# TimD1/vcfdist

Measured on AMD Instinct MI355X. Metric: supercluster-alignments/sec, higher is better.
Workload: dtype int32; 1 GPU; wgs_synth; superclusters_per_gpu=1000000, span_dist=lognormal(median 20, sigma 1.2) clip [4,10000]

## Files before the change

### vcfdist_amd/csrc/pr_api.hip

```cpp
#include <hip/hip_runtime.h>
#include <hip/hip_ext.h>
#include <dlfcn.h>

#include <algorithm>
#include <atomic>
#include <chrono>
#include <cstdarg>
#include <cstdio>
#include <cstdlib>
#include <cstring>
#include <condition_variable>
#include <deque>
#include <functional>
#include <mutex>
#include <string>
#include <thread>
#include <tuple>
#include <unordered_map>
#include <unordered_set>
#include <vector>

#include "../../include/vcfdist_pr.h"
#include "pr_device.h"
#include "pr_plan.h"
// ... 199 lines not shown
    if (lane == 0) wcnt[wave] = npop;
    __syncthreads();
    if (threadIdx.x == 0) {
        const int tot = wcnt[0] + wcnt[1] + wcnt[2] + wcnt[3];
        const int totp = pad4 ? ((tot + 3) & ~3) : tot;
        wbase = totp ? atomicAdd(cnt, totp) : 0;
        wtot = tot; wpad = totp - tot;
    }
    __syncthreads();
    int base = wbase;
    for (int w = 0; w < wave; w++) base += wcnt[w];
    if (bad) fail_list[base + __popcll(mbad & ((1ull << lane) - 1ull))] = a;
    if (int(threadIdx.x) < wpad) fail_list[wbase + wtot + int(threadIdx.x)] = -1;
}

__global__ void k_fails_count(const int32_t *__restrict__ work, int n, const AlnOut *__restrict__ outs, int32_t *__restrict__ blk,
                              int pad4, const int32_t *__restrict__ n_dev) {
    if (n_dev) n = min(n, *n_dev);
    const int i = blockIdx.x * blockDim.x + threadIdx.x;
    const int a = i < n ? work[i] : -1;
    const bool bad = a >= 0 && !outs[a].band_ok;
    const int npop = __popcll(__ballot(bad));
    __shared__ int wcnt[4];
    if ((threadIdx.x & 63) == 0) wcnt[threadIdx.x >> 6] = npop;
    __syncthreads();
    if (threadIdx.x == 0) {
        const int tot = wcnt[0] + wcnt[1] + wcnt[2] + wcnt[3];
        blk[blockIdx.x] = pad4 ? ((tot + 3) & ~3) : tot;
    }
}

#define FAILS_SCAN_NT 256
__global__ void __launch_bounds__(FAILS_SCAN_NT) k_fails_scan(int32_t *__restrict__ blk, int nb, int32_t *__restrict__ cnt) {
    __shared__ int32_t s_sum[FAILS_SCAN_NT];
    const int tid = threadIdx.x;
    const int per = (nb + FAILS_SCAN_NT - 1) / FAILS_SCAN_NT;
    const int b = min(nb, tid * per), e = min(nb, b + per);
    int32_t sum = 0;
    for (int k = b; k < e; k++) sum += blk[k];
    s_sum[tid] = sum;
    __syncthreads();
    for (int o = 1; o < FAILS_SCAN_NT; o <<= 1) {
        const int32_t v = tid >= o ? s_sum[tid - o] : 0;
        __syncthreads();
        s_sum[tid] += v;
        __syncthreads();
    }
    int32_t off = s_sum[tid] - sum;
    for (int k = b; k < e; k++) { const int32_t c = blk[k]; blk[k] = off; off += c; }
    if (tid == FAILS_SCAN_NT - 1) *cnt = s_sum[FAILS_SCAN_NT - 1];
}

__global__ void k_fails_scatter(const int32_t *__restrict__ work, int n, const AlnOut *__restrict__ outs, const int32_t *__restrict__ blk,
                                int32_t *__restrict__ fail_list, int pad4, const int32_t *__restrict__ n_dev) {
    if (n_dev) n = min(n, *n_dev);
    const int i = blockIdx.x * blockDim.x + threadIdx.x;
    const int a = i < n ? work[i] : -1;
    const bool bad = a >= 0 && !outs[a].band_ok;
    const unsigned long long mbad = __ballot(bad);
    const int lane = threadIdx.x & 63, wave = threadIdx.x >> 6;
    __shared__ int wcnt[4];
    if (lane == 0) wcnt[wave] = __popcll(mbad);
    __syncthreads();
    const int tot = wcnt[0] + wcnt[1] + wcnt[2] + wcnt[3];
    const int totp = pad4 ? ((tot + 3) & ~3) : tot;
    const int wbase = blk[blockIdx.x];
    int base = wbase;
    for (int w = 0; w < wave; w++) base += wcnt[w];
    if (bad) fail_list[base + __popcll(mbad & ((1ull << lane) - 1ull))] = a;
    if (int(threadIdx.x) < totp - tot) fail_list[wbase + tot + int(threadIdx.x)] = -1;
}

__global__ void k_publish_fails(const int32_t *__restrict__ list, const int32_t *__restrict__ cnt, int32_t *__restrict__ h_list,
                                int32_t *__restrict__ h_cnt, int copy_list) {
    const int n = *cnt;
    if (copy_list)
        for (int i = blockIdx.x * blockDim.x + threadIdx.x; i < n; i += gridDim.x * blockDim.x) h_list[i] = list[i];
    if (blockIdx.x == 0 && threadIdx.x == 0) *h_cnt = n;
    __threadfence_system();
}
// ... 6 lines not shown
    const AlnDesc d = src[i];
    dst[d.sc * 4 + d.aln] = d;
    dst_work[i] = src_work[i];
}

__global__ void k_collect_ties(const AlnOut *__restrict__ outs, int n, int4 *__restrict__ list, int32_t *__restrict__ cnt, int cap) {
    const int i = blockIdx.x * blockDim.x + threadIdx.x;
    if (i >= n) return;
    const int b = outs[i].band_ok;
    if (b >= 0) return;
    const int k = atomicAdd(cnt, 1);
    if (k < cap) list[k] = make_int4(i, -b - 1, outs[i].n_sec, outs[i].s);
}

__global__ void k_collect_ties_list(const int32_t *__restrict__ work, int n, const AlnOut *__restrict__ outs, int4 *__restrict__ list,
                                    int32_t *__restrict__ cnt, int cap) {
    const int i = blockIdx.x * blockDim.x + threadIdx.x;
    if (i >= n) return;
    const int a = work[i];
    if (a < 0) return;
    const int b = outs[a].band_ok;
    if (b >= 0) return;
    const int k = atomicAdd(cnt, 1);
    if (k < cap) list[k] = make_int4(a, -b - 1, outs[a].n_sec, outs[a].s);
}
__global__ void k_collect_spec(const int32_t *__restrict__ work, int n, const AlnOut *__restrict__ outs, int tag, int4 *__restrict__ list,
                               int32_t *__restrict__ cnt, int cap) {
    const int i = blockIdx.x * blockDim.x + threadIdx.x;
    if (i >= n) return;
    const int a = work[i];
    if (a < 0) return;
// ... 1344 lines not shown
    double phase_ms[6] = {0, 0, 0, 0, 0, 0};
    void phase(int k) { phase_ms[k] = std::chrono::duration<double, std::milli>(std::chrono::steady_clock::now() - call0).count(); }
    void lapx(const char *what) {
        if (h->debug) fprintf(stderr, "[vpr] execute %-34s %8.3f ms\n", what,
                              std::chrono::duration<double, std::milli>(std::chrono::steady_clock::now() - wall0).count());
    }

    void post_flag(int idx, hipStream_t ks) {
        flag_exp[idx] = ++h->flag_seq;
        hipLaunchKernelGGL(k_flag, dim3(1), dim3(1), 0, ks, h->hp_flag + idx, flag_exp[idx]);
        const hipError_t e = hipGetLastError();
        if (e != hipSuccess && launch_err == hipSuccess) launch_err = e;
    }
    hipError_t launch_err = hipSuccess;
    int64_t zl_wave0 = 0, zl_rows = 0;

    int idle_check(int64_t idle_polls, std::chrono::steady_clock::time_point since) {
        if (launch_err != hipSuccess) return fail(h, VPR_ERR_DEVICE, "kernel launch failed: %s", hipGetErrorString(launch_err));
        if (idle_polls % 2048) return VPR_OK;
        hipStream_t ss[] = {h->stream, h->cls_stream[0], h->cls_stream[1], h->cls_stream[2], h->cls_stream[3], h->cls_stream[4],
                            h->cls_stream[5], h->cls_stream[6], h->cls_stream[7],
                            h->tie_stream[0], h->tie_stream[1], h->tie_stream[2], h->tie_stream[3]};
        bool busy = false;
        for (hipStream_t s_ : ss) {
            const hipError_t e = hipStreamQuery(s_);
            if (e != hipSuccess && e != hipErrorNotReady) return fail(h, VPR_ERR_DEVICE, "stream error while waiting for a round: %s", hipGetErrorString(e));
            busy = busy || e == hipErrorNotReady;
        }
        const double idle_s = std::chrono::duration<double>(std::chrono::steady_clock::now() - since).count();
        static const double limit_s = [] { const char *e = getenv("VPR_IDLE_TIMEOUT_S"); const double v = e ? atof(e) : 0.0; return v > 0 ? v : 1800.0; }();
// ... 441 lines not shown
            restore = true;
            for (int32_t k = 0; k < cnt && restore; k++) {
                const auto it = tie_early.find(P.work[size_t(off) + size_t(k)]);
                if (it == tie_early.end() || it->second.plan != &h->plan0 || (it->second.mode != 1 && it->second.mode != 3) ||
                    it->second.pos < tie_resident->work_off || it->second.pos >= tie_resident->work_off + tie_resident->n_long) { restore = false; break; }
                const AlnDesc od = plan_desc(h, h->plan0, size_t(it->second.pos)), nd = plan_desc(h, P, size_t(off) + size_t(k));
                if (od.band_pad != LV_TAG[LV_C1] || od.pitch[0] != nd.pitch[0] || od.pitch[1] != nd.pitch[1] ||
                    od.mat_off[1] + int64_t(od.pitch[1]) * od.Lt > h->save_bytes) { restore = false; break; }
                rjobs[k] = RestoreJob{{od.mat_off[0], od.mat_off[1]}, od.blo_off};
            }
        }
        rc = timed(1, ls, ks, restore ? "k_restore_stripe" : band_fwd_name(lv), [&] {
            if (zero)
                hipExtLaunchKernelGGL(k_zero_lane, dim3((cnt + 63) / 64), dim3(64), h->zl_lds_bytes, ks, own_a, own_b, 0, h->d_descs, list, cnt,
                                      h->d_zl_hdr + zl_wave0, h->d_zl_in, h->d_zl_log, h->d_outs, a_path,
                                      (h->cfg.flags & VPR_CFG_KEEP_PATHS) ? 1 : 0, h->d_d1_hdr ? h->d1_max_rows : 0, h->lane_prio_rows);
            else if (q16)
                hipLaunchKernelGGL(k_fwd_q16, dim3((cnt + 3) / 4), dim3(64), 0, ks, h->dB, h->d_descs, list, cnt,
                                   P.arena, a_i32, h->d_outs, n_dev);
            else if (restore)
                hipLaunchKernelGGL(k_restore_stripe, dim3(cnt), dim3(256), 0, ks, h->d_descs, list, rjobs, h->plan0.arena,
                                   int64_t(reinterpret_cast<intptr_t>(h->d_save) - reinterpret_cast<intptr_t>(h->plan0.arena)), P.arena, a_i32);
            else if (save)
                hipLaunchKernelGGL(k_fwd_stripe_save, dim3(cnt), dim3(64), 0, ks, h->dB, h->d_descs, list, P.arena, a_i32, h->d_outs,
                                   fwd_save_delta);
            else
                hipLaunchKernelGGL(band_fwd_kernel(lv), dim3(cnt), dim3(lv >= LV_C4 ? W : 64), 0,
                                   ks, h->dB, h->d_descs, list, P.arena, a_i32, h->d_outs);
            hipLaunchKernelGGL(k_fwd_band_finish, dim3((cnt + 255) / 256), dim3(256), 0, ks, list, cnt, h->d_outs, tag, n_dev);
        }, zero);
        if (rc) return rc;
        n_fwd++;
        {
            const int32_t nc = n_dev ? n_all : cnt;
            if (zero && h->d_d1_blk) ordered_fails(list, nc, h->d_fail + fail_off, h->d_cnt + slot, n_dev, ks);
            else
            hipLaunchKernelGGL(k_collect_fails, dim3((nc + 255) / 256), dim3(256), 0, ks, list, nc, h->d_outs,
                               h->d_fail + fail_off, h->d_cnt + slot, zero ? 1 : 0, n_dev);
            hipLaunchKernelGGL(k_publish_fails, dim3(zero ? 1 : std::min((nc + 255) / 256, 1024)), dim3(256), 0, ks,
                               h->d_fail + fail_off, h->d_cnt + slot, h->hp_fail + fail_off, h->hp_cnt + slot, zero ? 0 : 1);
        }
        HIPCHK(h, hipEventRecord(h->ev_slot[slot], ks));
        }
        if ((phases & 2) && !zero) {
        ls.bytes_algorithmic = ls.cells;
        rc = timed(2, ls, ks, band_bwd_name(lv), [&] {
            if (q16)
                hipLaunchKernelGGL(k_bwd_q16, dim3((cnt + 3) / 4), dim3(64), 0, ks, h->dB, h->d_descs, list, cnt,
                                   P.arena, a_i32, h->d_outs, tag, dtag, n_dev);
            else
                hipLaunchKernelGGL(band_bwd_kernel(lv), dim3(cnt), dim3(lv >= LV_C4 ? W : 64), 0,
                                   ks, h->dB, h->d_descs, list, P.arena, a_i32, h->d_outs, tag);
        });
        if (rc) return rc;
        }
// ... 97 lines not shown
                if (wave_credit)
                    hipLaunchKernelGGL(k_credit<true>, dim3(cnt), dim3(64), 0, ks, h->dB, h->d_descs, list, cnt,
                                       h->d_outs, a_path, h->d_secs, h->d_fp_table, h->d_jobs, h->d_njobs,
                                       h->jobs_cap, dtag, tag, n_dev);
                else
                    hipLaunchKernelGGL(k_credit<false>, dim3((cnt + 63) / 64), dim3(64), 0, ks, h->dB, h->d_descs,
                                       list, cnt, h->d_outs, a_path, h->d_secs, h->d_fp_table, h->d_jobs,
                                       h->d_njobs, h->jobs_cap, dtag, tag, n_dev);
            });
        } else {
            rc = walk_launch(P, list, cnt, ks, wave_walk, tag);
        }
        return rc;
    }

    void ordered_fails(const int32_t *list, int32_t nc, int32_t *out, int32_t *cnt, const int32_t *n_dev, hipStream_t ks) {
        const int nb = (nc + 255) / 256;
        hipLaunchKernelGGL(k_fails_count, dim3(nb), dim3(256), 0, ks, list, nc, h->d_outs, h->d_d1_blk, 1, n_dev);
        hipLaunchKernelGGL(k_fails_scan, dim3(1), dim3(FAILS_SCAN_NT), 0, ks, h->d_d1_blk, nb, cnt);
        hipLaunchKernelGGL(k_fails_scatter, dim3(nb), dim3(256), 0, ks, list, nc, h->d_outs, h->d_d1_blk, out, 1, n_dev);
    }

    int enqueue_d1(const int32_t *list, const int32_t *n_dev, int32_t cap, int32_t n_all, hipStream_t ks, int ph, int ztag) {
        const int nw = (cap + 63) / 64;
        vpr_launch_stat ls;
        memset(&ls, 0, sizeof(ls));
        ls.threads = 64; ls.cells_per_thread = 1; ls.n_units = cap;
        int rc = VPR_OK;
        if (ph == 1) {
            rc = timed(0, ls, ks, "k_prep_d1", [&] {
                hipLaunchKernelGGL(k_d1_hdr, dim3(nw), dim3(64), 0, ks, h->d_descs, list, n_dev, cap, h->d_outs, h->d_d1_hdr);
                hipLaunchKernelGGL(k_d1_scan, dim3(1), dim3(D1_SCAN_NT), 0, ks, h->d_d1_hdr, nw, h->d1_in_cap, h->d1_log_cap, h->d_d1_info);
                hipLaunchKernelGGL(k_prep_d1, dim3(nw), dim3(256), 0, ks, h->dB, h->d_descs, list, n_dev, cap, h->d_outs, h->d_d1_hdr, h->d_d1_in);
            });
            if (rc) return rc;
            rc = timed(1, ls, ks, "k_one_lane", [&] {
                hipLaunchKernelGGL(k_one_lane, dim3(nw), dim3(64), 0, ks, h->d_descs, list, n_dev, cap, h->d_d1_hdr, h->d_d1_in, h->d_d1_log,
                                   h->d_outs, reinterpret_cast<PathEnt *>(h->plan0.arena), (h->cfg.flags & VPR_CFG_KEEP_PATHS) ? 1 : 0, h->d_d1_info,
                                   std::max(1, h->lane_prio_rows / 4));
                hipLaunchKernelGGL(k_fwd_band_finish, dim3((cap + 255) / 256), dim3(256), 0, ks, list, cap, h->d_outs, D1_TAG, n_dev);
            });
            if (rc) return rc;
            ordered_fails(list, n_all, h->d_d1_fail, h->d_d1_info + 2, n_dev, ks);
        } else if (ph == 4) {
            ls.cells_per_thread = 3;
            rc = timed(3, ls, ks, "k_one_tail", [&] {
                hipLaunchKernelGGL(k_one_tail, dim3(nw), dim3(64), 0, ks, h->dB, h->d_descs, list, n_dev, cap, h->d_d1_hdr, h->d_d1_in, h->d_d1_log,
                                   h->d_outs, reinterpret_cast<PathEnt *>(h->plan0.arena), (h->cfg.flags & VPR_CFG_KEEP_PATHS) ? 1 : 0, h->d_d1_info,
                                   h->d_secs, h->d_fp_table, h->d_jobs, h->d_njobs, h->jobs_cap, ztag, std::max(1, h->lane_prio_rows / 4));
            });
        }
        return rc;
    }

    int read_fails(int slot, int64_t fail_off, hipStream_t ls, std::vector<int32_t> &fails) {
        HIPCHK(h, x_event_sync(h, h->ev_slot[slot], SITE));
        const int32_t nf = h->hp_cnt[slot];
        if (nf > 0) {
// ... 26 lines not shown
            if (rc) return rc;
        }
        c.pending.clear();
        c.plans.clear();
        c.slot_cur = 0; c.fail_cur = 0;
        if (!overlap(c)) { c.stage_cur = 0; c.arena_cur = 0; }
        return VPR_OK;
    }

    int lad_tie_off(int k) { return h->tie_list_cap / 2 + k * (h->tie_list_cap / 4); }

    int lad_tie_cap(int k) { (void)k; return h->tie_list_cap / 4; }

    void ladder_collect(int k, const int32_t *list, int32_t n, hipStream_t ks) {
        hipLaunchKernelGGL(k_collect_ties_list, blocks(n), dim3(256), 0, ks, list, n, h->d_outs, h->d_tie_list + lad_tie_off(k),
                           h->d_tie_cnt + 5 + k, lad_tie_cap(k));
        hipLaunchKernelGGL(k_publish_ties, dim3(4), dim3(256), 0, ks, h->d_tie_list + lad_tie_off(k), h->d_tie_cnt + 5 + k,
                           h->hp_tie_list + lad_tie_off(k), h->hp_tie_cnt + 5 + k, lad_tie_cap(k));
        post_flag(9 + k, ks);
        lad_tie_wait[k] = true;
    }

    void drop_resident(const LadderCtx &c) {
        for (auto &r : h->resident)
            if (r.second >= c.arena && r.second < c.arena + c.arena_bytes) r.second = nullptr;
    }

    bool lad_grow(LadderCtx &c, int64_t nb, int64_t must = 0) {
        const int k = int(&c - h->lad);
        for (int j = 0; j < 4; j++) {
            LadderCtx &g = h->lad[j];
// ... 267 lines not shown
        tie_full = false;
        if (h->debug) fprintf(stderr, "[vpr] speculative replays: %d long alignments\n", n);
        int rc_ = tie_replay(spec_plan, 0, n, LT.ls, true);
        if (rc_) return rc_;
        spec_slot = tie_patch_slot; spec_off = tie_patch_off; spec_cap = tie_patch_cap;
        tie_patch_slot = -1;
        HIPCHK(h, hipEventRecord(h->ev_spec, LT.ls2));
        (void)hipStreamQuery(LT.ls2);
        for (int32_t k = 0; k < n; k++) spec_set[lst[k].x] = 1;
        tie_early.clear();
        tie_job_blocks.emplace_back(h->hp_tie_jobs + j0, tie_job_cur - j0);
        tie_job_total += tie_job_cur - j0;
        return VPR_OK;
    }

    int collect_part(int k, const int32_t *list, int32_t n, hipStream_t ks) {
        hipLaunchKernelGGL(k_collect_ties_list, blocks(n), dim3(256), 0, ks, list, n, h->d_outs, h->d_tie_list + tie_off[k],
                           h->d_tie_cnt + 2 + k, tie_cap[k]);
        hipLaunchKernelGGL(k_publish_ties, dim3(4), dim3(256), 0, ks, h->d_tie_list + tie_off[k], h->d_tie_cnt + 2 + k,
                           h->hp_tie_list + tie_off[k], h->hp_tie_cnt + 2 + k, tie_cap[k]);
        post_flag(2 + k, ks);
        return VPR_OK;
    }

    int round0_windowed() {
        int rc = VPR_OK;
        LL.ls = h->cls_stream[2]; LS.ls = h->cls_stream[3];
        LL.ls2 = h->cls_stream[5]; LS.ls2 = h->cls_stream[6]; LL.ev2 = h->ev_side[0]; LS.ev2 = h->ev_side[1];
        LL.slot0 = 2; LS.slot0 = 2 + LadderCtx::N_SLOTS;
        for (size_t ci = 0; ci < P0.chunks.size(); ci++) {
            const Chunk &ch = P0.chunks[ci];
            const int32_t n_long = ch.n_long;
            LL.arena_cur = LS.arena_cur = 0; LL.stage_cur = LS.stage_cur = 0;
            const int64_t rbase = na_ + na_ / 16 + 256;
            LL.fail_base = rbase; LS.fail_base = rbase + n_long;
            HIPCHK(h, hipMemsetAsync(h->d_cnt, 0, 8, st));
            if (ci == 0 && h->d_d1_info) HIPCHK(h, hipMemsetAsync(h->d_d1_info, 0, 64, st));
            HIPCHK(h, hipMemsetAsync(h->d_tie_cnt, 0, 32, st));
            HIPCHK(h, hipMemsetAsync(h->d_tie_ndec, 0, TIE_DEC_SLOTS * 4, st));
            tie_dec_slot = 0; tie_dec_cur = 0; tie_patch_slot = -1; spec_slot = -1;
            HIPCHK(h, hipEventRecord(h->ev_fork, st));
            HIPCHK(h, hipStreamWaitEvent(s_long, h->ev_fork, 0));
            HIPCHK(h, hipStreamWaitEvent(s_short, h->ev_fork, 0));
            HIPCHK(h, hipStreamWaitEvent(LL.ls, h->ev_fork, 0));
            HIPCHK(h, hipStreamWaitEvent(LS.ls, h->ev_fork, 0));
            for (int k = 0; k < 4; k++) HIPCHK(h, hipStreamWaitEvent(h->tie_stream[k], h->ev_fork, 0));
            for (int k = 2; k < 4; k++)
                for (int e = 0; e < 2; e++) {
                    LadderCtx &c = h->lad[k];
                    c.tie_clean[e] = 0;
                    if (ci == 0 && c.tie_scratch[e] && c.tie_first[e] > 0 && c.tie_first[e] <= c.tie_scratch_bytes[e]) {
// ... 11 lines not shown
            const bool inplace = P0.lv == LV_Z && n_short > 0;
            const int32_t *short_list = P0.d_work + ch.work_off + n_long;
            if (n_short > 0 && !inplace) {
                for (int ph = 1; ph <= 4; ph <<= 1) {
                    if ((rc = enqueue_part(P0, P0.d_work, ch.work_off + n_long, n_short, P0.lv, s_short, 1, n_long, false,
                                           ch.part_cells[1], ch.part_in[1], ch.part_dense[1], -1, ph))) return rc;
                    if (ph == 1) post_flag(1, s_short);
                    if (ph == 2 && (rc = collect_part(1, short_list, n_short, s_short))) return rc;
                }
            }
            if (inplace) {
                zl_wave0 = h->zl_wave0[ci];
                zl_rows = ch.part_rows[1];
                const int32_t *n_dev = h->d_cnt + 1;
                const int ztag = LV_TAG[LV_Z];
                HIPCHK(h, hipMemsetAsync(h->d_cnt + SLOT_IP, 0, 4, s_short));
                const bool d1 = h->d_d1_hdr != nullptr && cap_ip <= h->d1_wave_cap * 64;
                const int32_t n_all1 = n_short + n_short / 16 + 64;
                if (d1) HIPCHK(h, hipMemsetAsync(h->d_d1_info + 2, 0, 4, s_short));
                hipStream_t s_cred = h->side_credit ? h->cls_stream[7] : s_short;
                for (int ph = 1; ph <= 4; ph <<= 1) {
                    if (ph != 4 || s_cred == s_short) {
                        if ((rc = enqueue_part(P0, P0.d_work, ch.work_off + n_long, n_short, LV_Z, s_short, 1, n_long, false,
                                               ch.part_cells[1], ch.part_in[1], ch.part_dense[1], -1, ph))) return rc;
                        if (d1 && (rc = enqueue_d1(h->d_fail + n_long, n_dev, cap_ip, n_all1, s_short, ph, ztag))) return rc;
                    }
                    if (ph == 1 && s_cred != s_short) {
                        HIPCHK(h, hipEventRecord(h->ev_cred[0], s_short));
                        HIPCHK(h, hipStreamWaitEvent(s_cred, h->ev_cred[0], 0));
                        if ((rc = enqueue_part(P0, P0.d_work, ch.work_off + n_long, n_short, LV_Z, s_cred, 1, n_long, false,
                                               ch.part_cells[1], ch.part_in[1], ch.part_dense[1], -1, 4))) return rc;
                        if (d1 && (rc = enqueue_d1(h->d_fail + n_long, n_dev, cap_ip, n_all1, s_cred, 4, ztag))) return rc;
                        HIPCHK(h, hipEventRecord(h->ev_cred[1], s_cred));
                    }
                    if (ph == 4 && s_cred != s_short) HIPCHK(h, hipStreamWaitEvent(s_short, h->ev_cred[1], 0));
                    if ((rc = d1 ? enqueue_part(P0, h->d_d1_fail, 0, cap_ip, LV_Q16, s_short, SLOT_IP, foff_ip, false, 0, 0, 0,
                                                ztag, ph, h->d_d1_info + 2, std::min<int32_t>(h->d1_fail_cap, n_all1 + n_all1 / 64 + 64))
                                 : enqueue_part(P0, h->d_fail, n_long, cap_ip, LV_Q16, s_short, SLOT_IP, foff_ip, false, 0, 0, 0,
                                                ztag, ph, n_dev, n_all1))) return rc;
                    if (ph == 1) post_flag(1, s_short);
                    if (ph == 2 && (rc = collect_part(1, short_list, n_short, s_short))) return rc;
                }
            }
            if (n_long > 0) {
                const int lv = P0.lv <= LV_Q16 ? LONG_LV : P0.lv;
                for (int ph = 1; ph <= 4; ph <<= 1) {
                    fwd_save_delta = (ph == 1 && lv == LV_C1 && h->d_save) ? int64_t(reinterpret_cast<intptr_t>(h->d_save) - reinterpret_cast<intptr_t>(P0.arena)) : 0;
                    rc = enqueue_part(P0, P0.d_work, ch.work_off, n_long, lv, s_long, 0, 0, true, ch.part_cells[0],
                                      ch.part_in[0], ch.part_dense[0], -1, ph);
                    fwd_save_delta = 0;
                    if (rc) return rc;
                    if (ph == 1) {
                        post_flag(0, s_long);
                        if (lv == LV_C1) {
                            hipLaunchKernelGGL(k_collect_spec, blocks(n_long), dim3(256), 0, s_long, P0.d_work + ch.work_off, n_long, h->d_outs,
                                               LV_TAG[LV_C1], h->d_tie_list + tie_off[2], h->d_tie_cnt + 4, tie_cap[2]);
// ... 481 lines not shown
```

### vcfdist_amd/csrc/pr_d1.hip

```cpp
#ifndef PR_D1_HIP_
#define PR_D1_HIP_

#define D1_TAG 9
#define D1_CLEAN ZL_CLEAN_REJECT

#define GE_ALIVE 1u
#define GE_MAT 2u
#define GE_SWP 4u
#define GE_PSLOT_SHIFT 3
#define GE_SUB 32u
#define GE_SUB_SHIFT 6
#define GE_INS 256u
#define GE_INS_SHIFT 9
#define GE_DEL 2048u
#define GE_DEL_SHIFT 12
#define GE_TP 16384u
#define GE_BWD 32768u

#define MV_SWP_R 0
#define MV_MAT 1
#define MV_SUB 2
#define MV_INS 3
#define MV_DEL 4
#define MV_SWP_Q 5
// ... 124 lines not shown
                tile[lane][l] = v;
            }
            __syncthreads();
            const int rows = min(64, mlen - x0);
            for (int r = sub; r < rows; r += 4) out[int64_t(x0 + r) * 64 + lane] = tile[r][lane];
            __syncthreads();
        }
        out += int64_t(mlen) * 64;
    }
}

__global__ void __launch_bounds__(64, 3) k_one_lane(const AlnDesc *__restrict__ descs, const int32_t *__restrict__ list,
                                                    const int32_t *__restrict__ n_dev, int n_cap, const ZlWave *__restrict__ hdr,
                                                    const uint32_t *__restrict__ zin, uint4 *__restrict__ zlog,
                                                    AlnOut *__restrict__ outs, PathEnt *__restrict__ paths, int keep_paths,
                                                    int32_t *__restrict__ info, int prio_rows) {
    const int w = blockIdx.x, lane = threadIdx.x;
    const ZlWave H = hdr[w];
    if (H.mt <= 0) return;
    if (H.mt >= prio_rows) __builtin_amdgcn_s_setprio(2);
    const int n_list = min(*n_dev, n_cap);
    const int wi = w * 64 + lane;
    int a_ = wi < n_list ? list[wi] : -1;
    if (a_ >= 0 && outs[a_].exit_min != D1_CLEAN) a_ = -1;
    const bool live = a_ >= 0;
    {
        const int nl = __popcll(__ballot(live));
        if (lane == 0 && nl) atomicAdd(info + 3, nl);
    }
    const int a = max(a_, 0);
    const AlnDesc *dp = descs + a;
    const int Lq = live ? dp->Lq : 1, Lr = live ? dp->Lr : 1, Lt = live ? dp->Lt : 0;
    const int L[2] = {Lq, Lr};
    const auto rin = __builtin_amdgcn_make_buffer_rsrc(const_cast<uint32_t *>(zin + H.in_off), 0, 256 * (2 * H.mq + 2 * H.mr + H.mt), 0x00020000);
    const auto rlog = __builtin_amdgcn_make_buffer_rsrc(zlog + H.log_off, 0, 2560 * (H.mt + 1), 0x00020000);
    const uint32_t lane4 = uint32_t(lane) << 2, lane8 = uint32_t(lane) << 3, lane16 = uint32_t(lane) << 4;
    const uint32_t posW[2] = {0u, uint32_t(2 * H.mq) << 8}, posC[2] = {uint32_t(H.mq) << 8, uint32_t(2 * H.mq + H.mr) << 8};
    const uint32_t post = uint32_t(2 * H.mq + 2 * H.mr) << 8;
    const uint32_t logB1 = uint32_t(H.mt + 1) << 10, logB2 = logB1 + (uint32_t(H.mt + 1) << 9);
    auto in_at = [&](uint32_t off) -> uint32_t { return __builtin_amdgcn_raw_buffer_load_b32(rin, off, 0, 0); };
    auto word_at = [&](int p, int x, bool on) -> uint32_t { return in_at(on ? posW[p] + (uint32_t(x) << 8) + lane4 : ZL_OOB); };
    auto t_at = [&](int t, bool on) -> uint32_t { return in_at(on ? post + (uint32_t(t) << 8) + lane4 : ZL_OOB); };
    bool ok = live && Lt >= 2;
    const int rows = ok ? Lt : 0;
    int tmax = rows;
#pragma unroll
    for (int o = 32; o; o >>= 1) tmax = max(tmax, __shfl_xor(tmax, o));
    if (tmax == 0) return;
    using S2 = std::integral_constant<int, 2>;
    using S4 = std::integral_constant<int, 4>;
#ifdef D1_CLOCKS
    long long ck0 = wall_clock64();
    auto lapck = [&](int k) { const long long c = wall_clock64(); if (lane == 0) { atomicMax(info + 8 + k, int(c - ck0)); } ck0 = c; };
#else
    auto lapck = [&](int) {};
#endif

    int brow0 = 1 << 30;
    {
        int bq[2][4];
#pragma unroll
        for (int p = 0; p < 2; p++) {
#pragma unroll
// ... 78 lines not shown
            if (!__any(act)) continue;
            const uint32_t tw1 = t_at(t, act), tw0 = t_at(t - 1, act);
            const bool upper = act && (bq[0][2] >= 0 || bq[0][3] >= 0 || bq[1][2] >= 0 || bq[1][3] >= 0);
#ifdef D1_CLOCKS
            n_rows_++;
            if (__any(upper)) n_s4_++;
#endif
            if (__any(upper) || !b0_row(S2{}, t, act, tw1, tw0)) (void)b0_row(S4{}, t, act, tw1, tw0);
        }
#ifdef D1_CLOCKS
        if (lane == 0) { atomicAdd(info + 12, n_rows_); atomicAdd(info + 13, n_s4_); }
#endif
    }
    { const int c_ = __popcll(__ballot(ok)); if (lane == 0 && c_) atomicAdd(info + 5, c_); }
    lapck(0);
    if (!__any(ok)) return;

    {
        int fq[2][4], gq[2][4];
        uint32_t fw[2][4], gw[2][4];
#pragma unroll
        for (int p = 0; p < 2; p++) {
#pragma unroll
            for (int s = 0; s < 4; s++) { fq[p][s] = -1; fw[p][s] = 0; gq[p][s] = -1; gw[p][s] = 0; }
        }
        uint32_t tw0 = 0;
        auto fg_row = [&](auto Sc, int t, bool act, uint32_t tw1, const zl_u4 bp) -> bool {
            constexpr int S = decltype(Sc)::value;
            const uint32_t Tb = ZW_BASE(tw1);
            const bool t_allow = zw_fwd_allow(tw0);
            int nq[2][S];
// ... 152 lines not shown
            const zl_u4 bp = bp_n;
            bp_n = b_row(t + 1);
            tw_n = t_at(t + 1, ok && t + 1 < rows);
            bool upper = act && ((bp.y | bp.w) != 0u);
#pragma unroll
            for (int p = 0; p < 2; p++) upper = upper || (act && (fq[p][2] >= 0 || fq[p][3] >= 0 || gq[p][2] >= 0 || gq[p][3] >= 0));
            if (__any(upper) || !fg_row(S2{}, t, act, tw1, bp)) (void)fg_row(S4{}, t, act, tw1, bp);
        }
        { const int c_ = __popcll(__ballot(ok)); if (lane == 0 && c_) atomicAdd(info + 6, c_); }
        ok = ok && gq[0][0] == Lq - 1;
        { const int c_ = __popcll(__ballot(ok)); if (lane == 0 && c_) atomicAdd(info + 7, c_); }
    }
    lapck(1);
    if (live) {
        AlnOut &o = outs[a];
        o.dist_q = ok ? 1 : D_INF;
        o.dist_r = D_INF;
        o.exit_min = ok ? D_INF : 0;
    }
    if (!__any(ok)) return;

    const int nrow = ok ? Lt : 0;
    int bmax = nrow;
#pragma unroll
    for (int o = 32; o; o >>= 1) bmax = max(bmax, __shfl_xor(bmax, o));
    int beg_plane = VPR_PLANE_REF;
    {
        int kf[2][4], kg[2][4];
        uint32_t cf[2] = {0, 0};
        uint32_t cg[2][2] = {{0, 0}, {0, 0}};
#pragma unroll
        for (int p = 0; p < 2; p++) {
#pragma unroll
// ... 253 lines not shown
```

### vcfdist_amd/csrc/pr_zl.hip

```cpp
#ifndef PR_ZL_HIP_
#define PR_ZL_HIP_
#include <type_traits>


#define ZW_PTR(w) (int((w) & 0xffffu) - 1)
#define ZW_BASE(w) (((w) >> 16) & 0x7fu)
#define ZW_PV (1u << 23)
#define ZW_PB (1u << 24)
#define ZW_PE (1u << 25)
#define ZW_INS (1u << 26)
#define ZW_TP (1u << 27)
__device__ __forceinline__ bool zw_fwd_allow(uint32_t w) { return !(w & ZW_PV) || (w & ZW_PE); }
__device__ __forceinline__ bool zw_bwd_allow(uint32_t w) { return !(w & ZW_PV) || (w & ZW_PB); }

#define ZE_ALIVE 1u
#define ZE_HASMAT 2u
#define ZE_HASSWP 4u
#define ZE_PSLOT_SHIFT 3
#define ZE_TP 32u
#define ZE_BWD 64u

#define ZL_MAXLEN 65000
#define ZL_CLEAN_REJECT (-1)

// ... 53 lines not shown
            const int rows = min(64, mlen - x0);
            for (int r = sub; r < rows; r += 4) out[int64_t(x0 + r) * 64 + lane] = tile[r][lane];
            __syncthreads();
        }
        out += int64_t(mlen) * 64;
    }
}

typedef __attribute__((ext_vector_type(4))) unsigned int zl_u4;
typedef __attribute__((ext_vector_type(2))) unsigned int zl_u2;
#define ZL_OOB 0xfffffff0u

__global__ void __launch_bounds__(64, 6) k_zero_lane(const AlnDesc *__restrict__ descs, const int32_t *__restrict__ list, int n_list,
                                                  const ZlWave *__restrict__ hdr, const uint32_t *__restrict__ zin,
                                                  uint4 *__restrict__ zlog, AlnOut *__restrict__ outs, PathEnt *__restrict__ paths,
                                                  int keep_paths, int d1_max_rows, int prio_rows) {
    const int w = blockIdx.x, lane = threadIdx.x;
    const ZlWave H = hdr[w];
    if (H.mt >= prio_rows) __builtin_amdgcn_s_setprio(2);
    const int wi = w * 64 + lane;
    const int a_ = wi < n_list ? list[wi] : -1;
    const bool live = a_ >= 0;
    const int a = max(a_, 0);
    const AlnDesc *dp = descs + a;
    const int Lq = live ? dp->Lq : 1, Lr = live ? dp->Lr : 1, Lt = live ? dp->Lt : 0;
    const int L[2] = {Lq, Lr};
    const auto rin = __builtin_amdgcn_make_buffer_rsrc(const_cast<uint32_t *>(zin + H.in_off), 0, 256 * (H.mq + H.mr + H.mt), 0x00020000);
    const auto rlog = __builtin_amdgcn_make_buffer_rsrc(zlog + H.log_off, 0, 1280 * H.mt, 0x00020000);
    const uint32_t lane4 = uint32_t(lane) << 2, lane8 = uint32_t(lane) << 3;
    const uint32_t pos0[2] = {0u, uint32_t(H.mq) << 8}, post = uint32_t(H.mq + H.mr) << 8;
    const uint32_t logP0 = uint32_t(H.mt) << 9;
    auto in_at = [&](uint32_t off) -> uint32_t { return __builtin_amdgcn_raw_buffer_load_b32(rin, off, 0, 0); };
    bool ok = live && Lq < ZL_MAXLEN && Lr < ZL_MAXLEN && Lt < ZL_MAXLEN && Lt >= 2;
    const int rows = ok ? Lt : 0;
    int tmax = rows;
#pragma unroll
    for (int o = 32; o; o >>= 1) tmax = max(tmax, __shfl_xor(tmax, o));
    if (tmax == 0) {
        if (live) { outs[a].dist_q = D_INF; outs[a].dist_r = D_INF; outs[a].exit_min = 0; }
        return;
    }

    int qri[2][4];
    uint32_t pw[2][4];
#pragma unroll
    for (int p = 0; p < 2; p++) {
#pragma unroll
        for (int s = 0; s < 4; s++) { qri[p][s] = -1; pw[p][s] = 0; }
    }
    uint32_t tw0 = in_at(ok ? post + lane4 : ZL_OOB);
    if (ok) {
        qri[0][0] = 0; pw[0][0] = in_at(pos0[0] + lane4);
        qri[1][0] = 0; pw[1][0] = in_at(pos0[1] + lane4);
        zl_u2 e0;
// ... 107 lines not shown
#pragma unroll
        for (int p = 0; p < 2; p++) upper = upper || (act && (qri[p][2] >= 0 || qri[p][3] >= 0));
        if (__any(upper) || !fwd_row(std::integral_constant<int, 2>{}, t, act, tw1))
            (void)fwd_row(std::integral_constant<int, 4>{}, t, act, tw1);
    }
    int endq = -1, endr = -1;
#pragma unroll
    for (int s = 0; s < 4; s++) {
        if (qri[0][s] == Lq - 1) endq = s;
        if (qri[1][s] == Lr - 1) endr = s;
    }
    const bool clean = ok && Lt <= d1_max_rows;
    ok = ok && (endq >= 0 || endr >= 0);
    if (live) {
        AlnOut &o = outs[a];
        o.dist_q = (ok && endq >= 0) ? 0 : D_INF;
        o.dist_r = (ok && endr >= 0) ? 0 : D_INF;
        o.exit_min = ok ? D_INF : (clean ? ZL_CLEAN_REJECT : 0);
    }
    if (!__any(ok)) return;

    const int nrow = ok ? Lt : 0;
    int sc[2][4];
#pragma unroll
    for (int p = 0; p < 2; p++) {
#pragma unroll
        for (int s = 0; s < 4; s++) sc[p][s] = -1;
    }
    int bmax = nrow;
#pragma unroll
    for (int o = 32; o; o >>= 1) bmax = max(bmax, __shfl_xor(bmax, o));
    auto log_row = [&](int t, bool on) -> zl_u2 {
        return __builtin_amdgcn_raw_buffer_load_b64(rlog, on ? (uint32_t(t) << 9) + lane8 : ZL_OOB, 0, 0);
// ... 189 lines not shown
```

Before: 202.3 million supercluster-alignments/s.

## Fuse band-finish into lane kernels and drive fail compaction from reject bitmasks

Measured after the change: 201.6 million supercluster-alignments/s, median of 2. No clear change (-0.3%).

```diff
diff --git a/vcfdist_amd/csrc/pr_api.hip b/vcfdist_amd/csrc/pr_api.hip
--- a/vcfdist_amd/csrc/pr_api.hip
+++ b/vcfdist_amd/csrc/pr_api.hip
@@ -237,28 +237,36 @@
     if (int(threadIdx.x) < wpad) fail_list[wbase + wtot + int(threadIdx.x)] = -1;
 }
 
-__global__ void k_fails_count(const int32_t *__restrict__ work, int n, const AlnOut *__restrict__ outs, int32_t *__restrict__ blk,
-                              int pad4, const int32_t *__restrict__ n_dev) {
+#define FAILS_SCAN_NT 256
+__device__ __forceinline__ int fails_group_count(const unsigned long long *__restrict__ rej, const int32_t *__restrict__ work, int g,
+                                                 int n, int n_mask) {
+    int tot = 0;
+    if (g * 256 + 256 <= n_mask) {
+        const ulonglong2 *r2 = reinterpret_cast<const ulonglong2 *>(rej + g * 4);
+        const ulonglong2 u = r2[0], v = r2[1];
+        return (__popcll(u.x) + __popcll(u.y) + __popcll(v.x) + __popcll(v.y) + 3) & ~3;
+    }
+    for (int q = 0; q < 4; q++) {
+        const int i0 = (g * 4 + q) * 64;
+        if (i0 >= n) break;
+        if (i0 < n_mask) tot += __popcll(rej[g * 4 + q]);
+        for (int i = max(i0, n_mask); i < min(i0 + 64, n); i++) tot += work[i] >= 0 ? 1 : 0;
+    }
+    return (tot + 3) & ~3;
+}
+__global__ void __launch_bounds__(FAILS_SCAN_NT) k_fails_scan(const unsigned long long *__restrict__ rej, const int32_t *__restrict__ work,
+                                                              int n, int n_mask, const int32_t *__restrict__ n_dev,
+                                                              int32_t *__restrict__ blk, int32_t *__restrict__ cnt,
+                                                              int32_t *__restrict__ h_cnt, int32_t *__restrict__ zero) {
+    __shared__ int32_t s_sum[FAILS_SCAN_NT];
     if (n_dev) n = min(n, *n_dev);
-    const int i = blockIdx.x * blockDim.x + threadIdx.x;
-    const int a = i < n ? work[i] : -1;
-    const bool bad = a >= 0 && !outs[a].band_ok;
-    const int npop = __popcll(__ballot(bad));
-    __shared__ int wcnt[4];
-    if ((threadIdx.x & 63) == 0) wcnt[threadIdx.x >> 6] = npop;
-    __syncthreads();
-    if (threadIdx.x == 0) {
-        const int tot = wcnt[0] + wcnt[1] + wcnt[2] + wcnt[3];
-        blk[blockIdx.x] = pad4 ? ((tot + 3) & ~3) : tot;
-    }
-}
-
-#define FAILS_SCAN_NT 256
-__global__ void __launch_bounds__(FAILS_SCAN_NT) k_fails_scan(int32_t *__restrict__ blk, int nb, int32_t *__restrict__ cnt) {
-    __shared__ int32_t s_sum[FAILS_SCAN_NT];
+    n_mask = min(n_mask, n);
+    const int nb = (n + 255) / 256;
     const int tid = threadIdx.x;
     const int per = (nb + FAILS_SCAN_NT - 1) / FAILS_SCAN_NT;
     const int b = min(nb, tid * per), e = min(nb, b + per);
+    for (int k = tid; k < nb; k += FAILS_SCAN_NT) blk[k] = fails_group_count(rej, work, k, n, n_mask);
+    __syncthreads();
     int32_t sum = 0;
     for (int k = b; k < e; k++) sum += blk[k];
     s_sum[tid] = sum;
@@ -271,22 +279,29 @@
     }
     int32_t off = s_sum[tid] - sum;
     for (int k = b; k < e; k++) { const int32_t c = blk[k]; blk[k] = off; off += c; }
-    if (tid == FAILS_SCAN_NT - 1) *cnt = s_sum[FAILS_SCAN_NT - 1];
-}
-
-__global__ void k_fails_scatter(const int32_t *__restrict__ work, int n, const AlnOut *__restrict__ outs, const int32_t *__restrict__ blk,
-                                int32_t *__restrict__ fail_list, int pad4, const int32_t *__restrict__ n_dev) {
+    if (tid == FAILS_SCAN_NT - 1) {
+        const int32_t tot = s_sum[FAILS_SCAN_NT - 1];
+        *cnt = tot;
+        if (zero) *zero = 0;
+        if (h_cnt) { *h_cnt = tot; __threadfence_system(); }
+    }
+}
+
+__global__ void k_fails_scatter(const unsigned long long *__restrict__ rej, const int32_t *__restrict__ work, int n, int n_mask,
+                                const int32_t *__restrict__ n_dev, const int32_t *__restrict__ blk, int32_t *__restrict__ fail_list) {
     if (n_dev) n = min(n, *n_dev);
+    n_mask = min(n_mask, n);
+    if (int(blockIdx.x) * 256 >= n) return;
     const int i = blockIdx.x * blockDim.x + threadIdx.x;
     const int a = i < n ? work[i] : -1;
-    const bool bad = a >= 0 && !outs[a].band_ok;
+    const int lane = threadIdx.x & 63, wave = threadIdx.x >> 6;
+    const bool bad = i < n_mask ? ((rej[i >> 6] >> lane) & 1ull) != 0ull : a >= 0;
     const unsigned long long mbad = __ballot(bad);
-    const int lane = threadIdx.x & 63, wave = threadIdx.x >> 6;
     __shared__ int wcnt[4];
     if (lane == 0) wcnt[wave] = __popcll(mbad);
     __syncthreads();
     const int tot = wcnt[0] + wcnt[1] + wcnt[2] + wcnt[3];
-    const int totp = pad4 ? ((tot + 3) & ~3) : tot;
+    const int totp = (tot + 3) & ~3;
     const int wbase = blk[blockIdx.x];
     int base = wbase;
     for (int w = 0; w < wave; w++) base += wcnt[w];
@@ -323,7 +338,8 @@
 }
 
 __global__ void k_collect_ties_list(const int32_t *__restrict__ work, int n, const AlnOut *__restrict__ outs, int4 *__restrict__ list,
-                                    int32_t *__restrict__ cnt, int cap) {
+                                    int32_t *__restrict__ cnt, int cap, const int32_t *__restrict__ n_dev) {
+    if (n_dev) n = min(n, *n_dev);
     const int i = blockIdx.x * blockDim.x + threadIdx.x;
     if (i >= n) return;
     const int a = work[i];
@@ -1698,6 +1714,8 @@
     }
     hipError_t launch_err = hipSuccess;
     int64_t zl_wave0 = 0, zl_rows = 0;
+    unsigned long long *rej_z = nullptr, *rej_1 = nullptr;
+    int32_t *ip_cnt = nullptr;
 
     int idle_check(int64_t idle_polls, std::chrono::steady_clock::time_point since) {
         if (launch_err != hipSuccess) return fail(h, VPR_ERR_DEVICE, "kernel launch failed: %s", hipGetErrorString(launch_err));
@@ -2169,7 +2187,8 @@
             if (zero)
                 hipExtLaunchKernelGGL(k_zero_lane, dim3((cnt + 63) / 64), dim3(64), h->zl_lds_bytes, ks, own_a, own_b, 0, h->d_descs, list, cnt,
                                       h->d_zl_hdr + zl_wave0, h->d_zl_in, h->d_zl_log, h->d_outs, a_path,
-                                      (h->cfg.flags & VPR_CFG_KEEP_PATHS) ? 1 : 0, h->d_d1_hdr ? h->d1_max_rows : 0, h->lane_prio_rows);
+                                      (h->cfg.flags & VPR_CFG_KEEP_PATHS) ? 1 : 0, h->d_d1_hdr ? h->d1_max_rows : 0, h->lane_prio_rows, tag,
+                                      h->d_d1_blk ? rej_z : nullptr);
             else if (q16)
                 hipLaunchKernelGGL(k_fwd_q16, dim3((cnt + 3) / 4), dim3(64), 0, ks, h->dB, h->d_descs, list, cnt,
                                    P.arena, a_i32, h->d_outs, n_dev);
@@ -2182,18 +2201,19 @@
             else
                 hipLaunchKernelGGL(band_fwd_kernel(lv), dim3(cnt), dim3(lv >= LV_C4 ? W : 64), 0,
                                    ks, h->dB, h->d_descs, list, P.arena, a_i32, h->d_outs);
-            hipLaunchKernelGGL(k_fwd_band_finish, dim3((cnt + 255) / 256), dim3(256), 0, ks, list, cnt, h->d_outs, tag, n_dev);
+            if (!zero) hipLaunchKernelGGL(k_fwd_band_finish, dim3((cnt + 255) / 256), dim3(256), 0, ks, list, cnt, h->d_outs, tag, n_dev);
         }, zero);
         if (rc) return rc;
         n_fwd++;
         {
             const int32_t nc = n_dev ? n_all : cnt;
-            if (zero && h->d_d1_blk) ordered_fails(list, nc, h->d_fail + fail_off, h->d_cnt + slot, n_dev, ks);
-            else
+            if (zero && h->d_d1_blk && rej_z) ordered_fails(rej_z, list, nc, nc, h->d_fail + fail_off, h->d_cnt + slot, n_dev, ks, h->hp_cnt + slot, ip_cnt);
+            else {
             hipLaunchKernelGGL(k_collect_fails, dim3((nc + 255) / 256), dim3(256), 0, ks, list, nc, h->d_outs,
                                h->d_fail + fail_off, h->d_cnt + slot, zero ? 1 : 0, n_dev);
             hipLaunchKernelGGL(k_publish_fails, dim3(zero ? 1 : std::min((nc + 255) / 256, 1024)), dim3(256), 0, ks,
                                h->d_fail + fail_off, h->d_cnt + slot, h->hp_fail + fail_off, h->hp_cnt + slot, zero ? 0 : 1);
+            }
         }
         HIPCHK(h, hipEventRecord(h->ev_slot[slot], ks));
         }
@@ -2321,11 +2341,11 @@
         return rc;
     }
 
-    void ordered_fails(const int32_t *list, int32_t nc, int32_t *out, int32_t *cnt, const int32_t *n_dev, hipStream_t ks) {
+    void ordered_fails(const unsigned long long *rej, const int32_t *list, int32_t nc, int32_t n_mask, int32_t *out, int32_t *cnt,
+                       const int32_t *n_dev, hipStream_t ks, int32_t *h_cnt, int32_t *zero) {
         const int nb = (nc + 255) / 256;
-        hipLaunchKernelGGL(k_fails_count, dim3(nb), dim3(256), 0, ks, list, nc, h->d_outs, h->d_d1_blk, 1, n_dev);
-        hipLaunchKernelGGL(k_fails_scan, dim3(1), dim3(FAILS_SCAN_NT), 0, ks, h->d_d1_blk, nb, cnt);
-        hipLaunchKernelGGL(k_fails_scatter, dim3(nb), dim3(256), 0, ks, list, nc, h->d_outs, h->d_d1_blk, out, 1, n_dev);
+        hipLaunchKernelGGL(k_fails_scan, dim3(1), dim3(FAILS_SCAN_NT), 0, ks, rej, list, nc, n_mask, n_dev, h->d_d1_blk, cnt, h_cnt, zero);
+        hipLaunchKernelGGL(k_fails_scatter, dim3(nb), dim3(256), 0, ks, rej, list, nc, n_mask, n_dev, h->d_d1_blk, out);
     }
 
     int enqueue_d1(const int32_t *list, const int32_t *n_dev, int32_t cap, int32_t n_all, hipStream_t ks, int ph, int ztag) {
@@ -2344,11 +2364,10 @@
             rc = timed(1, ls, ks, "k_one_lane", [&] {
                 hipLaunchKernelGGL(k_one_lane, dim3(nw), dim3(64), 0, ks, h->d_descs, list, n_dev, cap, h->d_d1_hdr, h->d_d1_in, h->d_d1_log,
                                    h->d_outs, reinterpret_cast<PathEnt *>(h->plan0.arena), (h->cfg.flags & VPR_CFG_KEEP_PATHS) ? 1 : 0, h->d_d1_info,
-                                   std::max(1, h->lane_prio_rows / 4));
-                hipLaunchKernelGGL(k_fwd_band_finish, dim3((cap + 255) / 256), dim3(256), 0, ks, list, cap, h->d_outs, D1_TAG, n_dev);
+                                   std::max(1, h->lane_prio_rows / 4), D1_TAG, rej_1);
             });
             if (rc) return rc;
-            ordered_fails(list, n_all, h->d_d1_fail, h->d_d1_info + 2, n_dev, ks);
+            ordered_fails(rej_1, list, n_all, cap, h->d_d1_fail, h->d_d1_info + 2, n_dev, ks, nullptr, nullptr);
         } else if (ph == 4) {
             ls.cells_per_thread = 3;
             rc = timed(3, ls, ks, "k_one_tail", [&] {
@@ -2405,7 +2424,7 @@
 
     void ladder_collect(int k, const int32_t *list, int32_t n, hipStream_t ks) {
         hipLaunchKernelGGL(k_collect_ties_list, blocks(n), dim3(256), 0, ks, list, n, h->d_outs, h->d_tie_list + lad_tie_off(k),
-                           h->d_tie_cnt + 5 + k, lad_tie_cap(k));
+                           h->d_tie_cnt + 5 + k, lad_tie_cap(k), nullptr);
         hipLaunchKernelGGL(k_publish_ties, dim3(4), dim3(256), 0, ks, h->d_tie_list + lad_tie_off(k), h->d_tie_cnt + 5 + k,
                            h->hp_tie_list + lad_tie_off(k), h->hp_tie_cnt + 5 + k, lad_tie_cap(k));
         post_flag(9 + k, ks);
@@ -2703,9 +2722,9 @@
         return VPR_OK;
     }
 
-    int collect_part(int k, const int32_t *list, int32_t n, hipStream_t ks) {
+    int collect_part(int k, const int32_t *list, int32_t n, hipStream_t ks, const int32_t *n_dev = nullptr) {
         hipLaunchKernelGGL(k_collect_ties_list, blocks(n), dim3(256), 0, ks, list, n, h->d_outs, h->d_tie_list + tie_off[k],
-                           h->d_tie_cnt + 2 + k, tie_cap[k]);
+                           h->d_tie_cnt + 2 + k, tie_cap[k], n_dev);
         hipLaunchKernelGGL(k_publish_ties, dim3(4), dim3(256), 0, ks, h->d_tie_list + tie_off[k], h->d_tie_cnt + 2 + k,
                            h->hp_tie_list + tie_off[k], h->hp_tie_cnt + 2 + k, tie_cap[k]);
         post_flag(2 + k, ks);
@@ -2717,13 +2736,23 @@
         LL.ls = h->cls_stream[2]; LS.ls = h->cls_stream[3];
         LL.ls2 = h->cls_stream[5]; LS.ls2 = h->cls_stream[6]; LL.ev2 = h->ev_side[0]; LS.ev2 = h->ev_side[1];
         LL.slot0 = 2; LS.slot0 = 2 + LadderCtx::N_SLOTS;
+        rej_z = rej_1 = nullptr;
+        if (P0.lv == LV_Z && h->d_d1_blk) {
+            int64_t n_short_max = 0;
+            for (const Chunk &ch : P0.chunks) n_short_max = std::max<int64_t>(n_short_max, ch.count - ch.n_long);
+            const size_t nz = (size_t(n_short_max / 64 + 1) + 3) & ~size_t(3);
+            void *q = nullptr;
+            if (n_short_max > 0 && (rc = exec_alloc(h, &q, 2 * nz * sizeof(unsigned long long)))) return rc;
+            rej_z = static_cast<unsigned long long *>(q);
+            rej_1 = rej_z ? rej_z + nz : nullptr;
+        }
         for (size_t ci = 0; ci < P0.chunks.size(); ci++) {
             const Chunk &ch = P0.chunks[ci];
             const int32_t n_long = ch.n_long;
             LL.arena_cur = LS.arena_cur = 0; LL.stage_cur = LS.stage_cur = 0;
             const int64_t rbase = na_ + na_ / 16 + 256;
             LL.fail_base = rbase; LS.fail_base = rbase + n_long;
-            HIPCHK(h, hipMemsetAsync(h->d_cnt, 0, 8, st));
+            if (ci > 0) HIPCHK(h, hipMemsetAsync(h->d_cnt, 0, 8, st));
             if (ci == 0 && h->d_d1_info) HIPCHK(h, hipMemsetAsync(h->d_d1_info, 0, 64, st));
             HIPCHK(h, hipMemsetAsync(h->d_tie_cnt, 0, 32, st));
             HIPCHK(h, hipMemsetAsync(h->d_tie_ndec, 0, TIE_DEC_SLOTS * 4, st));
@@ -2765,10 +2794,10 @@
                 zl_rows = ch.part_rows[1];
                 const int32_t *n_dev = h->d_cnt + 1;
                 const int ztag = LV_TAG[LV_Z];
-                HIPCHK(h, hipMemsetAsync(h->d_cnt + SLOT_IP, 0, 4, s_short));
+                ip_cnt = (h->d_d1_blk && rej_z) ? h->d_cnt + SLOT_IP : nullptr;
+                if (!ip_cnt) HIPCHK(h, hipMemsetAsync(h->d_cnt + SLOT_IP, 0, 4, s_short));
                 const bool d1 = h->d_d1_hdr != nullptr && cap_ip <= h->d1_wave_cap * 64;
                 const int32_t n_all1 = n_short + n_short / 16 + 64;
-                if (d1) HIPCHK(h, hipMemsetAsync(h->d_d1_info + 2, 0, 4, s_short));
                 hipStream_t s_cred = h->side_credit ? h->cls_stream[7] : s_short;
                 for (int ph = 1; ph <= 4; ph <<= 1) {
                     if (ph != 4 || s_cred == s_short) {
@@ -2790,7 +2819,8 @@
                                  : enqueue_part(P0, h->d_fail, n_long, cap_ip, LV_Q16, s_short, SLOT_IP, foff_ip, false, 0, 0, 0,
                                                 ztag, ph, n_dev, n_all1))) return rc;
                     if (ph == 1) post_flag(1, s_short);
-                    if (ph == 2 && (rc = collect_part(1, short_list, n_short, s_short))) return rc;
+                    if (ph == 2 && (rc = d1 ? collect_part(1, h->d_d1_fail, cap_ip, s_short, h->d_d1_info + 2)
+                                            : collect_part(1, h->d_fail + n_long, cap_ip, s_short, n_dev))) return rc;
                 }
             }
             if (n_long > 0) {
diff --git a/vcfdist_amd/csrc/pr_d1.hip b/vcfdist_amd/csrc/pr_d1.hip
--- a/vcfdist_amd/csrc/pr_d1.hip
+++ b/vcfdist_amd/csrc/pr_d1.hip
@@ -162,14 +162,19 @@
                                                     const int32_t *__restrict__ n_dev, int n_cap, const ZlWave *__restrict__ hdr,
                                                     const uint32_t *__restrict__ zin, uint4 *__restrict__ zlog,
                                                     AlnOut *__restrict__ outs, PathEnt *__restrict__ paths, int keep_paths,
-                                                    int32_t *__restrict__ info, int prio_rows) {
+                                                    int32_t *__restrict__ info, int prio_rows, int tag,
+                                                    unsigned long long *__restrict__ rej) {
     const int w = blockIdx.x, lane = threadIdx.x;
     const ZlWave H = hdr[w];
-    if (H.mt <= 0) return;
-    if (H.mt >= prio_rows) __builtin_amdgcn_s_setprio(2);
     const int n_list = min(*n_dev, n_cap);
     const int wi = w * 64 + lane;
     int a_ = wi < n_list ? list[wi] : -1;
+    const unsigned long long m_in = __ballot(a_ >= 0);
+    if (H.mt <= 0) {
+        if (lane == 0) rej[w] = m_in;
+        return;
+    }
+    if (H.mt >= prio_rows) __builtin_amdgcn_s_setprio(2);
     if (a_ >= 0 && outs[a_].exit_min != D1_CLEAN) a_ = -1;
     const bool live = a_ >= 0;
     {
@@ -194,7 +199,10 @@
     int tmax = rows;
 #pragma unroll
     for (int o = 32; o; o >>= 1) tmax = max(tmax, __shfl_xor(tmax, o));
-    if (tmax == 0) return;
+    if (tmax == 0) {
+        if (lane == 0) rej[w] = m_in;
+        return;
+    }
     using S2 = std::integral_constant<int, 2>;
     using S4 = std::integral_constant<int, 4>;
 #ifdef D1_CLOCKS
@@ -303,7 +311,10 @@
     }
     { const int c_ = __popcll(__ballot(ok)); if (lane == 0 && c_) atomicAdd(info + 5, c_); }
     lapck(0);
-    if (!__any(ok)) return;
+    if (!__any(ok)) {
+        if (lane == 0) rej[w] = m_in;
+        return;
+    }
 
     {
         int fq[2][4], gq[2][4];
@@ -486,9 +497,19 @@
     lapck(1);
     if (live) {
         AlnOut &o = outs[a];
-        o.dist_q = ok ? 1 : D_INF;
-        o.dist_r = D_INF;
-        o.exit_min = ok ? D_INF : 0;
+        const int dq = ok ? 1 : D_INF, dr = D_INF;
+        const int em = ok ? D_INF : 0;
+        const int s = min(dq, dr);
+        o.dist_q = dq;
+        o.dist_r = dr;
+        o.exit_min = em;
+        o.s = s;
+        o.end_plane = (dq <= dr) ? VPR_PLANE_QUERY : VPR_PLANE_REF;
+        o.band_ok = (s < D_INF / 2 && em > s) ? tag : 0;
+    }
+    {
+        const unsigned long long mok = __ballot(ok);
+        if (lane == 0) rej[w] = m_in & ~mok;
     }
     if (!__any(ok)) return;
 
diff --git a/vcfdist_amd/csrc/pr_zl.hip b/vcfdist_amd/csrc/pr_zl.hip
--- a/vcfdist_amd/csrc/pr_zl.hip
+++ b/vcfdist_amd/csrc/pr_zl.hip
@@ -91,7 +91,8 @@
 __global__ void __launch_bounds__(64, 6) k_zero_lane(const AlnDesc *__restrict__ descs, const int32_t *__restrict__ list, int n_list,
                                                   const ZlWave *__restrict__ hdr, const uint32_t *__restrict__ zin,
                                                   uint4 *__restrict__ zlog, AlnOut *__restrict__ outs, PathEnt *__restrict__ paths,
-                                                  int keep_paths, int d1_max_rows, int prio_rows) {
+                                                  int keep_paths, int d1_max_rows, int prio_rows, int tag,
+                                                  unsigned long long *__restrict__ rej) {
     const int w = blockIdx.x, lane = threadIdx.x;
     const ZlWave H = hdr[w];
     if (H.mt >= prio_rows) __builtin_amdgcn_s_setprio(2);
@@ -114,7 +115,13 @@
 #pragma unroll
     for (int o = 32; o; o >>= 1) tmax = max(tmax, __shfl_xor(tmax, o));
     if (tmax == 0) {
-        if (live) { outs[a].dist_q = D_INF; outs[a].dist_r = D_INF; outs[a].exit_min = 0; }
+        if (live) {
+            AlnOut &o = outs[a];
+            o.dist_q = D_INF; o.dist_r = D_INF; o.exit_min = 0;
+            o.s = D_INF; o.end_plane = VPR_PLANE_QUERY; o.band_ok = 0;
+        }
+        const unsigned long long mrej = __ballot(live);
+        if (rej && lane == 0) rej[w] = mrej;
         return;
     }
 
@@ -252,9 +259,19 @@
     ok = ok && (endq >= 0 || endr >= 0);
     if (live) {
         AlnOut &o = outs[a];
-        o.dist_q = (ok && endq >= 0) ? 0 : D_INF;
-        o.dist_r = (ok && endr >= 0) ? 0 : D_INF;
-        o.exit_min = ok ? D_INF : (clean ? ZL_CLEAN_REJECT : 0);
+        const int dq = (ok && endq >= 0) ? 0 : D_INF, dr = (ok && endr >= 0) ? 0 : D_INF;
+        const int em = ok ? D_INF : (clean ? ZL_CLEAN_REJECT : 0);
+        const int s = min(dq, dr);
+        o.dist_q = dq;
+        o.dist_r = dr;
+        o.exit_min = em;
+        o.s = s;
+        o.end_plane = (dq <= dr) ? VPR_PLANE_QUERY : VPR_PLANE_REF;
+        o.band_ok = (s < D_INF / 2 && em > s) ? tag : 0;
+    }
+    {
+        const unsigned long long mrej = __ballot(live && !ok);
+        if (rej && lane == 0) rej[w] = mrej;
     }
     if (!__any(ok)) return;
 
```
